# his0si/ConvNet-Quantization

Measured on AMD Instinct MI355X. Metric: images/sec at batch 1024 (3×32×32) int8 static-PTQ, 1/2/4/8 MI355X; top-1 delta, higher is better.
Workload: dtype int8; 1 GPU; full static-PTQ SimpleConvNet, all conv+linear int8 (u8 x s8 -> i32), NHWC, per-tensor weights; global_batch=1024, per_gpu_batch=1024, parallelism=dp1

## Files before the change

### convnet-quantization_amd/csrc/conv3x3.hip

```cpp
#include "common.hpp"
#include "conv_epi.hpp"
#include "conv_launch.hpp"
#include <type_traits>
#include <utility>
#include <algorithm>
#include <cmath>
#include "qconvnet_abi.hpp"

namespace qcn {

constexpr int kPipeD = 2;
constexpr int kSm56D = 4;
constexpr int kProdPrio = 2;

template <int CIN, int COUT, int HW, bool POOL, int WPX, int PSP = 16, int RPAD = 0,
          int SPAD = 0, bool SPLIT = false, int WI_ = 2, int JT_ = 4, int RB_ = 0>
struct ConvCfg {
  static constexpr int kCin = CIN, kCout = COUT;
  static constexpr bool kPool = POOL, kSplit = SPLIT;
  static constexpr int W = HW, H = HW;
  static constexpr int WI = WI_;
  static constexpr int JT = JT_;
  static constexpr int MPS = JT * WI;
  static constexpr int kWpx = WPX;
// ... 1161 lines not shown
      const int PW = C::W / 2, PR = C::R / 2;
      const int q = wp * 32 + (j >> 2) * 16 + p, jq = j & 3;
      return slot(q / (PR * PW), 2 * ((q / PW) % PR) + (jq >> 1), 2 * (q % PW) + (jq & 1));
    }
    const int m = (wp * 8 + j) * 16 + p;
    return slot(m / (C::R * C::W), (m / C::W) % C::R, m % C::W);
  }
  template <class N>
  static constexpr int out_at(int wp, int j, int p) {
    const int m = (wp * 8 + j) * 16 + p;
    return Pix16<N>::slot(m / (C::R * C::W), (m / C::W) % C::R + 1, m % C::W + 1);
  }
  static constexpr int jofs(int j) { return at(0, j, 0) - at(0, 0, 0); }
  template <class N>
  static constexpr int out_jofs(int j) { return out_at<N>(0, j, 0) - out_at<N>(0, 0, 0); }
  static constexpr bool affine() {
    for (int wp = 0; wp < C::kWpx; ++wp)
      for (int j = 0; j < 8; ++j)
        for (int p = 0; p < 16; ++p)
          if (at(wp, j, p) != at(wp, 0, p) + jofs(j)) return false;
    return true;
  }
  template <class N>
  static constexpr bool out_affine() {
    for (int wp = 0; wp < C::kWpx; ++wp)
      for (int j = 0; j < 8; ++j)
        for (int p = 0; p < 16; ++p)
          if (out_at<N>(wp, j, p) != out_at<N>(wp, 0, p) + out_jofs<N>(j)) return false;
    return true;
  }
};

template <class C>
QCN_DEV void pipe_job16(const uint8_t* patch, const int* corr, wt_rsrc_t wr, wt_rsrc_t wrn, int voff, int wc,
                        int lb, int g, v4i (&acc)[4][8], v4i (&ga)[2][4]) {
  constexpr int CBK = C::kCin / 64, S = C::NCH;
  using X = Pix16<C>;
  static_assert(X::affine(), "pixel blocks at constant offsets");
  v4i c0[4];
#pragma unroll
  for (int i = 0; i < 4; ++i) c0[i] = *reinterpret_cast<const v4i*>(corr + wc * 64 + 16 * i + 4 * g);
  auto rd_b = [&](int s, int j) {
    const int tap = s / CBK, cb = s % CBK;
    return *reinterpret_cast<const v4i*>(patch + lb + X::jofs(j) + PatchAddr<C>::delta(tap, j) + cb * 64);
  };
  auto issue = [&](wt_rsrc_t r, int s, int slot) {
#pragma unroll
    for (int i = 0; i < 4; ++i) {
      const auto v = __builtin_amdgcn_raw_buffer_load_b128(r, voff, s * C::WBUF + i * 1024, 0);
      ga[slot][i] = (v4i){(int)v[0], (int)v[1], (int)v[2], (int)v[3]};
    }
  };
  v4i fb[8];
#pragma unroll
  for (int j = 0; j < 8; ++j) fb[j] = rd_b(0, j);
  static_for<S>([&](auto sc) {
    constexpr int s = decltype(sc)::value;
    static_for<32>([&](auto mc) {
      constexpr int m = decltype(mc)::value, j = m >> 2, i = m & 3;
      __builtin_amdgcn_sched_barrier(0);
      acc[i][j] = __builtin_amdgcn_mfma_i32_16x16x64_i8(ga[s & 1][i], fb[j], s == 0 ? c0[i] : acc[i][j], 0, 0, 0);
      __builtin_amdgcn_sched_barrier(0);
      if constexpr (m == 1 && s + 1 < S) {
        issue(wr, s + 1, (s + 1) & 1);
        __builtin_amdgcn_sched_barrier(0);
      }
      if constexpr (i == 3 && s + 1 < S) {
        fb[j] = rd_b(s + 1, j);
        __builtin_amdgcn_sched_barrier(0);
      }
    });
#pragma unroll
    for (int i = 0; i < 4; ++i)
#pragma unroll
      for (int j = 0; j < 8; ++j) asm volatile("" : "+v"(acc[i][j]));
  });
  issue(wrn, 0, 0);
  __builtin_amdgcn_sched_barrier(0);
}

template <class CA, class CB>
struct PairWs16 {
  static_assert(CA::NWAVES == 4 && CB::NWAVES == 4 && CA::WCO == CB::WCO && CA::WI == 2 && CB::WI == 2,
                "four waves of 64-cout x 128-pixel tiles per role");
  static_assert(!CA::kPool && CB::kPool && CA::kCout == CB::kCin, "A feeds B");
  static_assert(CA::PXB == CB::PXB && CA::SEGS == CB::SEGS && CA::R == CA::H && CA::W == CB::W &&
                !CA::kBand && !CB::kBand && !CA::kSplit, "whole images per tile");
  static_assert(Pix16<CA>::affine() && Pix16<CB>::affine() && Pix16<CA>::template out_affine<CB>(),
                "pixel blocks at constant offsets");
  static constexpr int SEGS = CA::SEGS, IMG = CA::IMG;
  static constexpr int IN_BYTES = SEGS * IMG * CA::kCin;
  static_assert(IN_BYTES == 4 * 256 * 16, "four 16-B staging pieces per A-role thread");
  static constexpr int PA = (CA::PATCH + 15) / 16 * 16, PB = (CB::PATCH + 15) / 16 * 16;
  static constexpr int TAB = 16 * (CA::kCout + CB::kCout);
  static constexpr bool DOUBLE_A = 2 * PA + 2 * PB + TAB <= 160 * 1024;
  static constexpr int OFF_PB = 0;
  static constexpr int OFF_PA = 2 * PB;
  static constexpr int OFF_EA = OFF_PA + (DOUBLE_A ? 2 : 1) * PA;
  static constexpr int OFF_EB = OFF_EA + 12 * CA::kCout;
  static constexpr int OFF_CA = OFF_EB + 12 * CB::kCout;
  static constexpr int OFF_CB = OFF_CA + 4 * CA::kCout;
  static constexpr int LDS = OFF_CB + 4 * CB::kCout;
  static_assert(LDS <= 160 * 1024, "LDS budget");
  static constexpr int OPI = CB::OPX / SEGS;
};

template <class CA, class CB, int FA, int FB, bool KMAJOR, bool ILV = false>
QCN_DEV void convpair_ws16_body(int b, int G, const uint8_t* __restrict__ x, int nimg, int x_zp,
                                const int8_t* __restrict__ wa, const ConvEpi& epa, int xb_zp,
                                const int8_t* __restrict__ wb, const ConvEpi& epb, uint8_t* __restrict__ y) {
  using P = PairWs16<CA, CB>;
  using XA = Pix16<CA>;
  using XB = Pix16<CB>;
  constexpr int SEGS = P::SEGS, IMG = CA::IMG, W = CA::W, WCO = CA::WCO;
  constexpr int CH16 = CA::kCin / 16;
  extern __shared__ __attribute__((aligned(16))) uint8_t lds[];
  const int tid = threadIdx.x;
  const int role = __builtin_amdgcn_readfirstlane(tid >> 8);
  const int rt = tid & 255, lane = tid & 63, wave = rt >> 6;
  const int wc = wave % WCO, wp = wave / WCO;
  int T;
  if constexpr (ILV) {
    const int mine = b < nimg ? (nimg - 1 - b) / G + 1 : 0;
    T = (mine + SEGS - 1) / SEGS;
  } else {
    const int ntile = (nimg + SEGS - 1) / SEGS;
    T = b < ntile ? (ntile - 1 - b) / G + 1 : 0;
  }
  auto img_of = [&](int k, int sg) {
    const int n = ILV ? b + (k * SEGS + sg) * G : (b + k * G) * SEGS + sg;
    return n < nimg ? n : (ILV ? b + k * SEGS * G : (b + k * G) * SEGS);
  };
  auto in_src = [&](int k, int q) {
    const int p = rt + 256 * q;
    const int n = img_of(k, p / (IMG * CH16));
    return x + ((long)n * IMG + (p / CH16) % IMG) * CA::kCin + (p % CH16) * 16;
  };
  auto in_dst = [&](int q) {
    const int p = rt + 256 * q;
    const int pix = (p / CH16) % IMG;
    return CA::slot(p / (IMG * CH16), pix / W + 1, pix % W + 1) + (p % CH16) * 16;
  };
  uint4 sv0[4];
  if (role == 0 && T > 0) {
#pragma unroll
    for (int q = 0; q < 4; ++q) sv0[q] = *reinterpret_cast<const uint4*>(in_src(0, q));
  }
  float* eka = reinterpret_cast<float*>(lds + P::OFF_EA);
  float* ekb = reinterpret_cast<float*>(lds + P::OFF_EB);
  int* cra = reinterpret_cast<int*>(lds + P::OFF_CA);
  int* crb = reinterpret_cast<int*>(lds + P::OFF_CB);
  constexpr int NA = 3 * CA::kCout / 4, NB = 3 * CB::kCout / 4;
  constexpr int NCA = CA::kCout / 4, NCB = CB::kCout / 4;
  constexpr int NTAB = NA + NB + NCA + NCB, TPT = (NTAB + 255) / 256;
  float4 tval[TPT];
  auto tab = [&](int e, bool dst) -> float4* {
    if (e < NA) {
      const int a = e / (CA::kCout / 4), o = e % (CA::kCout / 4);
      const float* s = a == 0 ? epa.u : (a == 1 ? epa.v : epa.mult);
      return dst ? reinterpret_cast<float4*>(eka) + e : const_cast<float4*>(reinterpret_cast<const float4*>(s) + o);
    }
    e -= NA;
    if (e < NB) {
      const int a = e / (CB::kCout / 4), o = e % (CB::kCout / 4);
      const float* s = a == 0 ? epb.u : (a == 1 ? epb.v : epb.mult);
      return dst ? reinterpret_cast<float4*>(ekb) + e : const_cast<float4*>(reinterpret_cast<const float4*>(s) + o);
    }
    e -= NB;
    if (e < NCA)
      return dst ? reinterpret_cast<float4*>(cra) + e
                 : const_cast<float4*>(reinterpret_cast<const float4*>(epa.corr) + e);
    e -= NCA;
    return dst ? reinterpret_cast<float4*>(crb) + e
               : const_cast<float4*>(reinterpret_cast<const float4*>(epb.corr) + e);
  };
  {
    const uint32_t pa4 = xor80(splat_u8(x_zp)), pb4 = xor80(splat_u8(xb_zp));
    auto halo = [&](auto cfg, uint8_t* base, int nbuf, int pbytes, uint32_t pad) {
      using C = decltype(cfg);
      constexpr int HS = 2 * C::PCOLS + 2 * (C::PROWS - 2), CH = C::kCin / 16;
      const int total = nbuf * C::SEGS * HS * CH;
      for (int e = tid; e < total; e += 512) {
        const int c = e % CH, hs = (e / CH) % HS, sg = (e / (CH * HS)) % C::SEGS, bf = e / (CH * HS * C::SEGS);
        int pr, pc;
        if (hs < C::PCOLS) { pr = 0; pc = hs; }
        else if (hs < 2 * C::PCOLS) { pr = C::PROWS - 1; pc = hs - C::PCOLS; }
        else { const int r = hs - 2 * C::PCOLS; pr = 1 + (r >> 1); pc = (r & 1) ? C::PCOLS - 1 : 0; }
        *reinterpret_cast<uint4*>(base + bf * pbytes + C::slot(sg, pr, pc) + c * 16) = make_uint4(pad, pad, pad, pad);
      }
    };
    halo(CA{}, lds + P::OFF_PA, P::DOUBLE_A ? 2 : 1, P::PA, pa4);
    halo(CB{}, lds + P::OFF_PB, 2, P::PB, pb4);
  }
  if (role == 1) {
#pragma unroll
    for (int k = 0; k < TPT; ++k)
      if (rt + 256 * k < NTAB) tval[k] = *tab(rt + 256 * k, false);
#pragma unroll
    for (int k = 0; k < TPT; ++k)
      if (rt + 256 * k < NTAB) *tab(rt + 256 * k, true) = tval[k];
  }
  if (T == 0) return;

  const int p16 = lane & 15, g = lane >> 4;
  const wt_rsrc_t wra = wt_rsrc(wa), wrb = wt_rsrc(wb);
  const int voff = (wc * 64 + p16) * 64 + g * 16;
  auto pa_buf = [&](int j) { return lds + P::OFF_PA + (P::DOUBLE_A ? (j & 1) * P::PA : 0); };
  auto pb_buf = [&](int j) { return lds + P::OFF_PB + (j & 1) * P::PB; };
  auto write_in = [&](uint8_t* pa, const uint4 (&sv)[4]) {
#pragma unroll
    for (int q = 0; q < 4; ++q)
      *reinterpret_cast<uint4*>(pa + in_dst(q)) =
          make_uint4(xor80(sv[q].x), xor80(sv[q].y), xor80(sv[q].z), xor80(sv[q].w));
  };
  auto first_chunk = [&](wt_rsrc_t w0, v4i (&ga)[2][4]) {
#pragma unroll
    for (int i = 0; i < 4; ++i) {
      const auto v = __builtin_amdgcn_raw_buffer_load_b128(w0, voff, i * 1024, 0);
      ga[0][i] = (v4i){(int)v[0], (int)v[1], (int)v[2], (int)v[3]};
    }
  };

  v4i acc[4][8];
  if (role == 0) write_in(pa_buf(0), sv0);
  lds_barrier();

  struct Lane {
    int p16, g, ek;
    int la, lb;
    int hb;
    int q;
    const int *ca, *cb;
  };
  auto lanes = [&]() {
    int lz = lane;
    asm volatile("" : "+v"(lz));
    Lane L;
    L.p16 = lz & 15;
    L.g = lz >> 4;
    L.ek = wc * 64 + 4 * L.g;
    L.la = XA::at(wp, 0, L.p16) + 16 * L.g;
    L.lb = XB::at(wp, 0, L.p16) + 16 * L.g;
    L.hb = XA::template out_at<CB>(wp, 0, L.p16) + wc * 64 + 4 * L.g;
    L.q = wp * 32 + L.p16;
    L.ca = cra + (lz >> 6);
    L.cb = crb + (lz >> 6);
    return L;
  };
  auto epi_a = [&](const Lane& L, uint8_t* pb) {
    static_for<4>([&](auto ic) {
      constexpr int i = decltype(ic)::value;
      const EpiG K = load_epig(eka, CA::kCout, L.ek + 16 * i);
      static_for<8>([&](auto jc) {
        constexpr int j = decltype(jc)::value;
        uint32_t wd = 0;
#pragma unroll
        for (int r = 0; r < 4; ++r) wd = rq_elem<FA>(acc[i][j][r], K, r, epa, wd);
        *reinterpret_cast<uint32_t*>(pb + L.hb + XA::template out_jofs<CB>(j) + 16 * i) = xor80(wd);
      });
    });
  };
  auto epi_b = [&](const Lane& L, int k) {
    static_for<2>([&](auto gc) {
      constexpr int gq = decltype(gc)::value;
      uint32_t d[4];
      static_for<4>([&](auto ic) {
        constexpr int i = decltype(ic)::value;
        const EpiG K = load_epig(ekb, CB::kCout, L.ek + 16 * i);
        uint32_t wd = 0;
#pragma unroll
        for (int r = 0; r < 4; ++r) {
          const int a = max(max(acc[i][4 * gq][r], acc[i][4 * gq + 1][r]),
                            max(acc[i][4 * gq + 2][r], acc[i][4 * gq + 3][r]));
          wd = rq_elem<FB>(a, K, r, epb, wd);
        }
        d[i] = wd;
      });
      const auto s02 = __builtin_amdgcn_permlane32_swap(d[0], d[2], false, false);
      const auto s13 = __builtin_amdgcn_permlane32_swap(d[1], d[3], false, false);
      const auto t01 = __builtin_amdgcn_permlane16_swap(s02[0], s13[0], false, false);
      const auto t23 = __builtin_amdgcn_permlane16_swap(s02[1], s13[1], false, false);
      const uint4 v = make_uint4(t01[0], t01[1], t23[0], t23[1]);
      const int q = L.q + 16 * gq;
      const int n = img_of(k, q / P::OPI), pix = q % P::OPI;
      const int co = wc * 64 + 16 * L.g;
      const bool real = ILV ? b + (k * SEGS + q / P::OPI) * G < nimg : (b + k * G) * SEGS + q / P::OPI < nimg;
      if (real) {
        if constexpr (KMAJOR) {
          const int kc = (pix * CB::kCout + co) / 32;
          store_wt16(wt_rsrc(y), (uint32_t)(((long)kc * nimg + n) * 32 + 16 * (L.g & 1)), v);
        } else {
          store_wt16(wt_rsrc(y + (long)n * P::OPI * CB::kCout), (uint32_t)(pix * CB::kCout + co), v);
        }
      }
    });
  };

  if (role == 0) {
    v4i ga[2][4];
    first_chunk(wra, ga);
    uint4 sv[4] = {};
#pragma unroll 1
    for (int p = 0; p <= T; ++p) {
      if constexpr (!P::DOUBLE_A) {
        if (p >= 1 && p < T) write_in(pa_buf(p), sv);
        lds_barrier();
      }
      WS16_STAMP(p, 0);
      if (p < T) {
        const Lane L = lanes();
        pipe_job16<CA>(pa_buf(p), L.ca, wra, wra, voff, wc, L.la, L.g, acc, ga);
        WS16_STAMP(p, 1);
        const int kn = p + 1 < T ? p + 1 : p;
#pragma unroll
        for (int q = 0; q < 4; ++q) sv[q] = *reinterpret_cast<const uint4*>(in_src(kn, q));
        epi_a(L, pb_buf(p));
        if constexpr (P::DOUBLE_A) write_in(pa_buf(p + 1), sv);
        WS16_STAMP(p, 2);
      }
      lds_barrier();
    }
  } else {
    v4i ga[2][4];
    first_chunk(wrb, ga);
#pragma unroll 1
    for (int p = 0; p <= T; ++p) {
      if constexpr (!P::DOUBLE_A) lds_barrier();
      WS16_STAMP(p, 0);
      if (p >= 1) {
        const Lane L = lanes();
        if (p >= 2) epi_b(L, p - 2);
        WS16_STAMP(p, 1);
        pipe_job16<CB>(pb_buf(p - 1), L.cb, wrb, wrb, voff, wc, L.lb, L.g, acc, ga);
        WS16_STAMP(p, 2);
      }
      lds_barrier();
    }
    const Lane L = lanes();
    epi_b(L, T - 1);
#ifdef QCN_CONVNET_STAMP
    if (T + 1 < 8) { WS16_STAMP(T + 1, 0); }
#endif
  }
}

template <class CA, class CB, int FA, int FB, bool KMAJOR>
__global__ __launch_bounds__(512, 1)
void convpair_ws16_kernel(const uint8_t* __restrict__ x, int nimg, int x_zp, const int8_t* __restrict__ wa,
                          ConvEpi epa, int xb_zp, const int8_t* __restrict__ wb, ConvEpi epb,
                          uint8_t* __restrict__ y) {
  convpair_ws16_body<CA, CB, FA, FB, KMAJOR>((int)blockIdx.x, (int)gridDim.x, x, nimg, x_zp, wa, epa, xb_zp,
                                             wb, epb, y);
}

using W16A3 = ConvCfg<64, 128, 16, false, 2, 32, 0, 0, false>;
using W16B4 = ConvCfg<128, 128, 16, true, 2, 32, 64, 0, true>;
using W16A5 = ConvCfg<128, 256, 8, false, 1, 32, 192, 0, false>;
using W16B6 = ConvCfg<256, 256, 8, true, 1, 32, 0, 0, true>;

struct Conv1Cfg {
  static constexpr int H = 32, W = 32, R = 16, COUT = 64, NT = 256;
  static constexpr int PXB = R * W;
  static constexpr int PR = R + 2, PC = W + 2;
  static constexpr int PATCH = 3 * PR * PC;
  static constexpr int PATCH_AL = (PATCH + 15) / 16 * 16;
  static constexpr int KS = 32 + 16;
  static constexpr int LDS = PATCH_AL + PXB * KS;
};

template <int HW>
__global__ __launch_bounds__(256, 3)
void conv1_f32_kernel(const float* __restrict__ x, int nimg, float in_inv, int in_zp,
                      const int8_t* __restrict__ w1, ConvEpi ep, uint8_t* __restrict__ y,
                      uint8_t* __restrict__ qin_out) {
  constexpr int H = HW, W = HW;
// ... 549 lines not shown
                    const int8_t* __restrict__ w1, ConvEpi ep1, int x2_zp,
                    const int8_t* __restrict__ w2, ConvEpi ep2, uint8_t* __restrict__ y) {
  const int T = (int)blockIdx.x < nimg ? 2 * ((nimg - 1 - (int)blockIdx.x) / (int)gridDim.x + 1) : 0;
  conv12p_body((int)blockIdx.x, (int)gridDim.x, T, x, nimg, in_inv, in_zp, w1, ep1, x2_zp, w2, ep2, y);
}
#endif

#define QCN_C16_PARAMS                                                                                   \
  const int8_t* __restrict__ w0, ConvEpi e0, int z0, const int8_t* __restrict__ w1, ConvEpi e1, int z1, \
      const int8_t* __restrict__ w2, ConvEpi e2, int z2, const int8_t* __restrict__ w3, ConvEpi e3,      \
      int z3, const int8_t* __restrict__ w4, ConvEpi e4, int z4, const int8_t* __restrict__ w5,          \
      ConvEpi e5, int z5
#define QCN_C16_ARGS(L)                                                                                  \
  (L).w[0], (L).ep[0], (L).x_zp[0], (L).w[1], (L).ep[1], (L).x_zp[1], (L).w[2], (L).ep[2], (L).x_zp[2],   \
      (L).w[3], (L).ep[3], (L).x_zp[3], (L).w[4], (L).ep[4], (L).x_zp[4], (L).w[5], (L).ep[5], (L).x_zp[5]

struct ConvnetLayers {
  const int8_t* w[6];
  ConvEpi ep[6];
  int x_zp[6];
};

using SmA3 = ConvCfg<64, 128, 16, false, 4, 16, 96, 0, false, 2, 2>;
using SmB4 = ConvCfg<128, 128, 16, true, 2, 16, 32, 0, true, 1, 4>;
using SmA5 = ConvCfg<128, 256, 8, false, 1, 16, 224, 0, false, 1, 2>;
using SmB6 = ConvCfg<256, 256, 8, true, 1, 16, 32, 64, true, 1, 2>;

using WsA3 = ConvCfg<64, 128, 16, false, 2, 16, 96, 0, false>;
using WsB4 = ConvCfg<128, 128, 16, true, 2, 16, 32, 0, true>;
using WsA5 = ConvCfg<128, 256, 8, false, 1, 16, 224, 0, false>;
using WsB6 = ConvCfg<256, 256, 8, true, 1, 16, 32, 64, true>;

constexpr int cmax(int a, int b) { return a > b ? a : b; }
constexpr int kConvnet16Lds = cmax(Conv12P::LDS, cmax(PairWs16<W16A3, W16B4>::LDS, PairWs16<W16A5, W16B6>::LDS));
constexpr int kConvnetSmLds = cmax(Conv12P::LDS, cmax(PairCfg<SmA3, SmB4>::LDS, PairGaCfg<SmA5, SmB6>::LDS));

#ifdef QCN_CONVNET_STAMP
__device__ unsigned long long g_c16_stamp[4096][8];
QCN_DEV void c16_stamp(int i) {
  const unsigned long long t = __builtin_amdgcn_s_memtime();
  const unsigned long long r = __builtin_amdgcn_s_memrealtime();
  const unsigned lane = __builtin_amdgcn_mbcnt_hi(~0u, __builtin_amdgcn_mbcnt_lo(~0u, 0u));
  if ((threadIdx.x >> 6) == 0 && lane == 0 && blockIdx.x < 4096) {
    volatile unsigned long long* d = g_c16_stamp[blockIdx.x];
    d[i] = t + lane;
    d[4 + i] = r + lane;
  }
}
#define C16_STAMP(i) c16_stamp(i)
#else
#define C16_STAMP(i)
#endif

QCN_DEV void phase_boundary() {
  asm volatile("s_waitcnt vmcnt(0) lgkmcnt(0)" ::: "memory");
  __builtin_amdgcn_s_setprio(0);
  __syncthreads();
}

template <int EM, bool KMAJOR>
__global__ __launch_bounds__(512, 1)
void convnet_convs16_kernel(const float* __restrict__ x, int nimg, float in_inv, QCN_C16_PARAMS,
                            uint8_t* __restrict__ a2, uint8_t* __restrict__ a4, uint8_t* __restrict__ a6) {
  static_assert(PairWs16<W16A3, W16B4>::SEGS == 1, "conv3+4 tile k of workgroup b is image b + kG");
  const int b = (int)blockIdx.x, G = (int)gridDim.x;
  const int T = b < nimg ? 2 * ((nimg - 1 - b) / G + 1) : 0;
  C16_STAMP(0);
  conv12p_body(b, G, T, x, nimg, in_inv, z0, w0, e0, z1, w1, e1, a2);
  phase_boundary();
  C16_STAMP(1);
  convpair_ws16_body<W16A3, W16B4, EM, EM, false>(b, G, a2, nimg, z2, w2, e2, z3, w3, e3, a4);
  phase_boundary();
  C16_STAMP(2);
  convpair_ws16_body<W16A5, W16B6, EM, EM, KMAJOR, true>(b, G, a4, nimg, z4, w4, e4, z5, w5, e5, a6);
#ifdef QCN_CONVNET_STAMP
  __syncthreads();
#endif
  C16_STAMP(3);
}

#ifndef QCN_CONV_U8_TU
__global__ __launch_bounds__(512, 1)
void convnet_convs_sm_kernel(const float* __restrict__ x, int nimg, float in_inv, QCN_C16_PARAMS,
                             uint8_t* __restrict__ a2, uint8_t* __restrict__ a4, uint8_t* __restrict__ a6) {
  const int b = (int)blockIdx.x;
  C16_STAMP(0);
  conv12p_body(b, (int)gridDim.x, 2, x, nimg, in_inv, z0, w0, e0, z1, w1, e1, a2);
  phase_boundary();
  C16_STAMP(1);
  convpair_body<SmA3, SmB4>(b, a2, nimg, z2, w2, e2, z3, w3, e3, a4);
  phase_boundary();
  C16_STAMP(2);
  convpair_ga_body<SmA5, SmB6, kSm56D>(b, a4, nimg, z4, w4, e4, z5, w5, e5, a6);
#ifdef QCN_CONVNET_STAMP
  __syncthreads();
#endif
  C16_STAMP(3);
}

struct ConvsF32 {
  static constexpr auto sm = convnet_convs_sm_kernel;
  template <int EM, bool KMAJOR>
  static constexpr auto k16 = convnet_convs16_kernel<EM, KMAJOR>;
  static constexpr int kLdsSm = kConvnetSmLds, kLds16 = kConvnet16Lds;
};
#endif

// ... 494 lines not shown
```

### convnet-quantization_amd/csrc/conv3x3_u8.hip

```cpp
#define QCN_CONV_U8_TU 1
#define QCN_NO_ABI 1
#include "conv3x3.hip"

namespace qcn {

constexpr int kConvnet16LdsU8 = cmax(Conv12P::LDS_U8, kConvnet16Lds);
constexpr int kConvnetSmLdsU8 = cmax(Conv12P::LDS_U8, kConvnetSmLds);

__global__ __launch_bounds__(512, 1)
void conv12p_u8_kernel(const uint8_t* __restrict__ img, int nimg, const uint8_t* __restrict__ qlut,
                       int in_zp, const int8_t* __restrict__ w1, ConvEpi ep1, int x2_zp,
                       const int8_t* __restrict__ w2, ConvEpi ep2, uint8_t* __restrict__ y) {
  const int T = (int)blockIdx.x < nimg ? 2 * ((nimg - 1 - (int)blockIdx.x) / (int)gridDim.x + 1) : 0;
  conv12p_body((int)blockIdx.x, (int)gridDim.x, T, img, nimg, 0.0f, in_zp, w1, ep1, x2_zp, w2, ep2, y,
               qlut);
}

template <int EM, bool KMAJOR>
__global__ __launch_bounds__(512, 1)
void convnet_convs16_u8_kernel(const uint8_t* __restrict__ img, int nimg,
                               const uint8_t* __restrict__ qlut, QCN_C16_PARAMS,
                               uint8_t* __restrict__ a2, uint8_t* __restrict__ a4,
                               uint8_t* __restrict__ a6) {
  static_assert(PairWs16<W16A3, W16B4>::SEGS == 1, "conv3+4 tile k of workgroup b is image b + kG");
  const int b = (int)blockIdx.x, G = (int)gridDim.x;
  const int T = b < nimg ? 2 * ((nimg - 1 - b) / G + 1) : 0;
  conv12p_body(b, G, T, img, nimg, 0.0f, z0, w0, e0, z1, w1, e1, a2, qlut);
  phase_boundary();
  convpair_ws16_body<W16A3, W16B4, EM, EM, false>(b, G, a2, nimg, z2, w2, e2, z3, w3, e3, a4);
  phase_boundary();
  convpair_ws16_body<W16A5, W16B6, EM, EM, KMAJOR, true>(b, G, a4, nimg, z4, w4, e4, z5, w5, e5, a6);
}

__global__ __launch_bounds__(512, 1)
void convnet_convs_sm_u8_kernel(const uint8_t* __restrict__ img, int nimg,
                                const uint8_t* __restrict__ qlut, QCN_C16_PARAMS,
                                uint8_t* __restrict__ a2, uint8_t* __restrict__ a4,
                                uint8_t* __restrict__ a6) {
  const int b = (int)blockIdx.x;
  conv12p_body(b, (int)gridDim.x, 2, img, nimg, 0.0f, z0, w0, e0, z1, w1, e1, a2, qlut);
  phase_boundary();
  convpair_body<SmA3, SmB4>(b, a2, nimg, z2, w2, e2, z3, w3, e3, a4);
  phase_boundary();
  convpair_ga_body<SmA5, SmB6, kSm56D>(b, a4, nimg, z4, w4, e4, z5, w5, e5, a6);
}

struct ConvsU8 {
  static constexpr auto sm = convnet_convs_sm_u8_kernel;
  template <int EM, bool KMAJOR>
  static constexpr auto k16 = convnet_convs16_u8_kernel<EM, KMAJOR>;
  static constexpr int kLdsSm = kConvnetSmLdsU8, kLds16 = kConvnet16LdsU8;
};

}

extern "C" {

int qcn_conv12_fused_u8_nhwc(const uint8_t* img, int nimg, const uint8_t* qlut, int in_zp,
                             const int8_t* w1_packed, const float* u1, const float* v1,
                             const float* mult1, const int32_t* corr1, int z1, int relu1,
                             const qcn_qdq_t* qdq1, int x2_zp, const int8_t* w2_packed,
                             const float* u2, const float* v2, const float* mult2,
                             const int32_t* corr2, int y_zp, int relu2, const qcn_qdq_t* qdq2,
                             uint8_t* y, void* stream) {
// ... 15 lines not shown
```

Measured before the change: 8.473 million images/sec.

## Overlap conv3+4 tail with conv5+6 prologue across the phase seam

```diff
diff --git a/convnet-quantization_amd/csrc/conv3x3.hip b/convnet-quantization_amd/csrc/conv3x3.hip
--- a/convnet-quantization_amd/csrc/conv3x3.hip
+++ b/convnet-quantization_amd/csrc/conv3x3.hip
@@ -1218,7 +1218,7 @@
 
 template <class C>
 QCN_DEV void pipe_job16(const uint8_t* patch, const int* corr, wt_rsrc_t wr, wt_rsrc_t wrn, int voff, int wc,
-                        int lb, int g, v4i (&acc)[4][8], v4i (&ga)[2][4]) {
+                        int lb, int g, v4i (&acc)[4][8], v4i (&ga)[2][4], bool drain = false) {
   constexpr int CBK = C::kCin / 64, S = C::NCH;
   using X = Pix16<C>;
   static_assert(X::affine(), "pixel blocks at constant offsets");
@@ -1260,6 +1260,7 @@
 #pragma unroll
       for (int j = 0; j < 8; ++j) asm volatile("" : "+v"(acc[i][j]));
   });
+  if (drain) asm volatile("s_waitcnt vmcnt(0)" ::: "memory");
   issue(wrn, 0, 0);
   __builtin_amdgcn_sched_barrier(0);
 }
@@ -1290,56 +1291,106 @@
   static constexpr int OPI = CB::OPX / SEGS;
 };
 
-template <class CA, class CB, int FA, int FB, bool KMAJOR, bool ILV = false>
-QCN_DEV void convpair_ws16_body(int b, int G, const uint8_t* __restrict__ x, int nimg, int x_zp,
-                                const int8_t* __restrict__ wa, const ConvEpi& epa, int xb_zp,
-                                const int8_t* __restrict__ wb, const ConvEpi& epb, uint8_t* __restrict__ y) {
+template <class CA, class CB, int FA, int FB, bool KMAJOR, bool ILV = false, int OFF_TAB = PairWs16<CA, CB>::OFF_EA>
+struct Ws16 {
   using P = PairWs16<CA, CB>;
   using XA = Pix16<CA>;
   using XB = Pix16<CB>;
-  constexpr int SEGS = P::SEGS, IMG = CA::IMG, W = CA::W, WCO = CA::WCO;
-  constexpr int CH16 = CA::kCin / 16;
-  extern __shared__ __attribute__((aligned(16))) uint8_t lds[];
-  const int tid = threadIdx.x;
-  const int role = __builtin_amdgcn_readfirstlane(tid >> 8);
-  const int rt = tid & 255, lane = tid & 63, wave = rt >> 6;
-  const int wc = wave % WCO, wp = wave / WCO;
-  int T;
-  if constexpr (ILV) {
-    const int mine = b < nimg ? (nimg - 1 - b) / G + 1 : 0;
-    T = (mine + SEGS - 1) / SEGS;
-  } else {
-    const int ntile = (nimg + SEGS - 1) / SEGS;
-    T = b < ntile ? (ntile - 1 - b) / G + 1 : 0;
-  }
-  auto img_of = [&](int k, int sg) {
+  static constexpr int SEGS = P::SEGS, IMG = CA::IMG, W = CA::W, WCO = CA::WCO;
+  static constexpr int CH16 = CA::kCin / 16;
+  static_assert(OFF_TAB % 16 == 0 && (OFF_TAB == P::OFF_EA || OFF_TAB >= P::LDS) && OFF_TAB + P::TAB <= 160 * 1024,
+                "the tables in their own place or above the phase's patches");
+  static constexpr int OFF_EA = OFF_TAB, OFF_EB = OFF_EA + 12 * CA::kCout, OFF_CA = OFF_EB + 12 * CB::kCout,
+                       OFF_CB = OFF_CA + 4 * CA::kCout;
+  static constexpr int NA = 3 * CA::kCout / 4, NB = 3 * CB::kCout / 4;
+  static constexpr int NCA = CA::kCout / 4, NCB = CB::kCout / 4;
+  static constexpr int NTAB = NA + NB + NCA + NCB, TPT = (NTAB + 255) / 256;
+
+  const int b, G;
+  const uint8_t* const x;
+  const int nimg, x_zp;
+  const ConvEpi& epa;
+  const int xb_zp;
+  const ConvEpi& epb;
+  uint8_t* const y;
+  const wt_rsrc_t wra, wrb;
+  uint8_t* lds;
+  int tid, role, rt, lane, wc, wp, voff, T;
+  float *eka, *ekb;
+  int *cra, *crb;
+
+  QCN_DEV Ws16(int b_, int G_, const uint8_t* x_, int nimg_, int x_zp_, const int8_t* wa, const ConvEpi& epa_,
+               int xb_zp_, const int8_t* wb, const ConvEpi& epb_, uint8_t* y_, bool fresh = false)
+      : b(b_), G(G_), x(x_), nimg(nimg_), x_zp(x_zp_), epa(epa_), xb_zp(xb_zp_), epb(epb_), y(y_),
+        wra(wt_rsrc(wa)), wrb(wt_rsrc(wb)) {
+    extern __shared__ __attribute__((aligned(16))) uint8_t lds_[];
+    lds = lds_;
+    tid = threadIdx.x;
+    if (fresh) asm volatile("" : "+v"(tid));
+    role = __builtin_amdgcn_readfirstlane(tid >> 8);
+    rt = tid & 255, lane = tid & 63;
+    const int wave = rt >> 6;
+    wc = wave % WCO, wp = wave / WCO;
+    voff = (wc * 64 + (lane & 15)) * 64 + (lane >> 4) * 16;
+    if constexpr (ILV) {
+      const int mine = b < nimg ? (nimg - 1 - b) / G + 1 : 0;
+      T = (mine + SEGS - 1) / SEGS;
+    } else {
+      const int ntile = (nimg + SEGS - 1) / SEGS;
+      T = b < ntile ? (ntile - 1 - b) / G + 1 : 0;
+    }
+    eka = reinterpret_cast<float*>(lds + OFF_EA);
+    ekb = reinterpret_cast<float*>(lds + OFF_EB);
+    cra = reinterpret_cast<int*>(lds + OFF_CA);
+    crb = reinterpret_cast<int*>(lds + OFF_CB);
+  }
+
+  QCN_DEV int img_of(int k, int sg) const {
     const int n = ILV ? b + (k * SEGS + sg) * G : (b + k * G) * SEGS + sg;
     return n < nimg ? n : (ILV ? b + k * SEGS * G : (b + k * G) * SEGS);
-  };
-  auto in_src = [&](int k, int q) {
+  }
+  QCN_DEV const uint8_t* in_src(int k, int q) const {
     const int p = rt + 256 * q;
     const int n = img_of(k, p / (IMG * CH16));
     return x + ((long)n * IMG + (p / CH16) % IMG) * CA::kCin + (p % CH16) * 16;
-  };
-  auto in_dst = [&](int q) {
+  }
+  QCN_DEV int in_dst(int q) const {
     const int p = rt + 256 * q;
     const int pix = (p / CH16) % IMG;
     return CA::slot(p / (IMG * CH16), pix / W + 1, pix % W + 1) + (p % CH16) * 16;
-  };
-  uint4 sv0[4];
-  if (role == 0 && T > 0) {
-#pragma unroll
-    for (int q = 0; q < 4; ++q) sv0[q] = *reinterpret_cast<const uint4*>(in_src(0, q));
-  }
-  float* eka = reinterpret_cast<float*>(lds + P::OFF_EA);
-  float* ekb = reinterpret_cast<float*>(lds + P::OFF_EB);
-  int* cra = reinterpret_cast<int*>(lds + P::OFF_CA);
-  int* crb = reinterpret_cast<int*>(lds + P::OFF_CB);
-  constexpr int NA = 3 * CA::kCout / 4, NB = 3 * CB::kCout / 4;
-  constexpr int NCA = CA::kCout / 4, NCB = CB::kCout / 4;
-  constexpr int NTAB = NA + NB + NCA + NCB, TPT = (NTAB + 255) / 256;
-  float4 tval[TPT];
-  auto tab = [&](int e, bool dst) -> float4* {
+  }
+  QCN_DEV void load_in(int k, uint4 (&sv)[4]) const {
+#pragma unroll
+    for (int q = 0; q < 4; ++q) sv[q] = *reinterpret_cast<const uint4*>(in_src(k, q));
+  }
+  QCN_DEV void write_in(uint8_t* pa, const uint4 (&sv)[4]) const {
+#pragma unroll
+    for (int q = 0; q < 4; ++q)
+      *reinterpret_cast<uint4*>(pa + in_dst(q)) =
+          make_uint4(xor80(sv[q].x), xor80(sv[q].y), xor80(sv[q].z), xor80(sv[q].w));
+  }
+  QCN_DEV uint8_t* pa_buf(int j) const { return lds + P::OFF_PA + (P::DOUBLE_A ? (j & 1) * P::PA : 0); }
+  QCN_DEV uint8_t* pb_buf(int j) const { return lds + P::OFF_PB + (j & 1) * P::PB; }
+
+  template <class C>
+  QCN_DEV void halo(uint8_t* base, int nbuf, int pbytes, uint32_t pad, int t, int n) const {
+    constexpr int HS = 2 * C::PCOLS + 2 * (C::PROWS - 2), CH = C::kCin / 16;
+    const int total = nbuf * C::SEGS * HS * CH;
+    for (int e = t; e < total; e += n) {
+      const int c = e % CH, hs = (e / CH) % HS, sg = (e / (CH * HS)) % C::SEGS, bf = e / (CH * HS * C::SEGS);
+      int pr, pc;
+      if (hs < C::PCOLS) { pr = 0; pc = hs; }
+      else if (hs < 2 * C::PCOLS) { pr = C::PROWS - 1; pc = hs - C::PCOLS; }
+      else { const int r = hs - 2 * C::PCOLS; pr = 1 + (r >> 1); pc = (r & 1) ? C::PCOLS - 1 : 0; }
+      *reinterpret_cast<uint4*>(base + bf * pbytes + C::slot(sg, pr, pc) + c * 16) = make_uint4(pad, pad, pad, pad);
+    }
+  }
+  QCN_DEV void halo_a(int t, int n) const {
+    halo<CA>(lds + P::OFF_PA, P::DOUBLE_A ? 2 : 1, P::PA, xor80(splat_u8(x_zp)), t, n);
+  }
+  QCN_DEV void halo_b(int t, int n) const { halo<CB>(lds + P::OFF_PB, 2, P::PB, xor80(splat_u8(xb_zp)), t, n); }
+
+  QCN_DEV float4* tab(int e, bool dst) const {
     if (e < NA) {
       const int a = e / (CA::kCout / 4), o = e % (CA::kCout / 4);
       const float* s = a == 0 ? epa.u : (a == 1 ? epa.v : epa.mult);
@@ -1358,26 +1409,9 @@
     e -= NCA;
     return dst ? reinterpret_cast<float4*>(crb) + e
                : const_cast<float4*>(reinterpret_cast<const float4*>(epb.corr) + e);
-  };
-  {
-    const uint32_t pa4 = xor80(splat_u8(x_zp)), pb4 = xor80(splat_u8(xb_zp));
-    auto halo = [&](auto cfg, uint8_t* base, int nbuf, int pbytes, uint32_t pad) {
-      using C = decltype(cfg);
-      constexpr int HS = 2 * C::PCOLS + 2 * (C::PROWS - 2), CH = C::kCin / 16;
-      const int total = nbuf * C::SEGS * HS * CH;
-      for (int e = tid; e < total; e += 512) {
-        const int c = e % CH, hs = (e / CH) % HS, sg = (e / (CH * HS)) % C::SEGS, bf = e / (CH * HS * C::SEGS);
-        int pr, pc;
-        if (hs < C::PCOLS) { pr = 0; pc = hs; }
-        else if (hs < 2 * C::PCOLS) { pr = C::PROWS - 1; pc = hs - C::PCOLS; }
-        else { const int r = hs - 2 * C::PCOLS; pr = 1 + (r >> 1); pc = (r & 1) ? C::PCOLS - 1 : 0; }
-        *reinterpret_cast<uint4*>(base + bf * pbytes + C::slot(sg, pr, pc) + c * 16) = make_uint4(pad, pad, pad, pad);
-      }
-    };
-    halo(CA{}, lds + P::OFF_PA, P::DOUBLE_A ? 2 : 1, P::PA, pa4);
-    halo(CB{}, lds + P::OFF_PB, 2, P::PB, pb4);
-  }
-  if (role == 1) {
+  }
+  QCN_DEV void tables() const {
+    float4 tval[TPT];
 #pragma unroll
     for (int k = 0; k < TPT; ++k)
       if (rt + 256 * k < NTAB) tval[k] = *tab(rt + 256 * k, false);
@@ -1385,30 +1419,26 @@
     for (int k = 0; k < TPT; ++k)
       if (rt + 256 * k < NTAB) *tab(rt + 256 * k, true) = tval[k];
   }
-  if (T == 0) return;
-
-  const int p16 = lane & 15, g = lane >> 4;
-  const wt_rsrc_t wra = wt_rsrc(wa), wrb = wt_rsrc(wb);
-  const int voff = (wc * 64 + p16) * 64 + g * 16;
-  auto pa_buf = [&](int j) { return lds + P::OFF_PA + (P::DOUBLE_A ? (j & 1) * P::PA : 0); };
-  auto pb_buf = [&](int j) { return lds + P::OFF_PB + (j & 1) * P::PB; };
-  auto write_in = [&](uint8_t* pa, const uint4 (&sv)[4]) {
-#pragma unroll
-    for (int q = 0; q < 4; ++q)
-      *reinterpret_cast<uint4*>(pa + in_dst(q)) =
-          make_uint4(xor80(sv[q].x), xor80(sv[q].y), xor80(sv[q].z), xor80(sv[q].w));
-  };
-  auto first_chunk = [&](wt_rsrc_t w0, v4i (&ga)[2][4]) {
+
+  QCN_DEV bool prologue() const {
+    uint4 sv0[4];
+    if (role == 0 && T > 0) load_in(0, sv0);
+    halo_a(tid, 512);
+    halo_b(tid, 512);
+    if (role == 1) tables();
+    if (T == 0) return false;
+    if (role == 0) write_in(pa_buf(0), sv0);
+    lds_barrier();
+    return true;
+  }
+
+  QCN_DEV void first_chunk(wt_rsrc_t w0, v4i (&ga)[2][4]) const {
 #pragma unroll
     for (int i = 0; i < 4; ++i) {
       const auto v = __builtin_amdgcn_raw_buffer_load_b128(w0, voff, i * 1024, 0);
       ga[0][i] = (v4i){(int)v[0], (int)v[1], (int)v[2], (int)v[3]};
     }
-  };
-
-  v4i acc[4][8];
-  if (role == 0) write_in(pa_buf(0), sv0);
-  lds_barrier();
+  }
 
   struct Lane {
     int p16, g, ek;
@@ -1417,7 +1447,7 @@
     int q;
     const int *ca, *cb;
   };
-  auto lanes = [&]() {
+  QCN_DEV Lane lanes() const {
     int lz = lane;
     asm volatile("" : "+v"(lz));
     Lane L;
@@ -1431,8 +1461,8 @@
     L.ca = cra + (lz >> 6);
     L.cb = crb + (lz >> 6);
     return L;
-  };
-  auto epi_a = [&](const Lane& L, uint8_t* pb) {
+  }
+  QCN_DEV void epi_a(const Lane& L, uint8_t* pb, const v4i (&acc)[4][8]) const {
     static_for<4>([&](auto ic) {
       constexpr int i = decltype(ic)::value;
       const EpiG K = load_epig(eka, CA::kCout, L.ek + 16 * i);
@@ -1444,8 +1474,8 @@
         *reinterpret_cast<uint32_t*>(pb + L.hb + XA::template out_jofs<CB>(j) + 16 * i) = xor80(wd);
       });
     });
-  };
-  auto epi_b = [&](const Lane& L, int k) {
+  }
+  QCN_DEV void epi_b(const Lane& L, int k, const v4i (&acc)[4][8]) const {
     static_for<2>([&](auto gc) {
       constexpr int gq = decltype(gc)::value;
       uint32_t d[4];
@@ -1479,53 +1509,72 @@
         }
       }
     });
-  };
-
-  if (role == 0) {
+  }
+  QCN_DEV void stamp(int p, int k) const { WS16_STAMP(p, k); }
+
+  QCN_DEV void period_a(int p, uint4 (&sv)[4], v4i (&acc)[4][8], v4i (&ga)[2][4], bool seam = false) const {
+    if constexpr (!P::DOUBLE_A) {
+      if (p >= 1 && p < T) write_in(pa_buf(p), sv);
+      lds_barrier();
+    }
+    stamp(p, 0);
+    if (p < T) {
+      const Lane L = lanes();
+      pipe_job16<CA>(pa_buf(p), L.ca, wra, wra, voff, wc, L.la, L.g, acc, ga);
+      stamp(p, 1);
+      load_in(!seam && p + 1 < T ? p + 1 : p, sv);
+      if (seam) lds_barrier();
+      epi_a(L, pb_buf(p), acc);
+      if constexpr (P::DOUBLE_A) write_in(pa_buf(p + 1), sv);
+      stamp(p, 2);
+    }
+    lds_barrier();
+    if (seam) {
+      int k = p + 1 < T ? p + 1 : p;
+      asm volatile("" : "+v"(k));
+      load_in(__builtin_amdgcn_readfirstlane(k), sv);
+    }
+  }
+  QCN_DEV void period_b(int p, v4i (&acc)[4][8], v4i (&ga)[2][4], bool drain = false) const {
+    if constexpr (!P::DOUBLE_A) lds_barrier();
+    stamp(p, 0);
+    if (p >= 1) {
+      const Lane L = lanes();
+      if (p >= 2) epi_b(L, p - 2, acc);
+      stamp(p, 1);
+      pipe_job16<CB>(pb_buf(p - 1), L.cb, wrb, wrb, voff, wc, L.lb, L.g, acc, ga, drain);
+      stamp(p, 2);
+    }
+    lds_barrier();
+  }
+  QCN_DEV void last_epi_b(const v4i (&acc)[4][8]) const {
+    const Lane L = lanes();
+    epi_b(L, T - 1, acc);
+#ifdef QCN_CONVNET_STAMP
+    if (T + 1 < 8) stamp(T + 1, 0);
+#endif
+  }
+};
+
+template <class CA, class CB, int FA, int FB, bool KMAJOR, bool ILV = false>
+QCN_DEV void convpair_ws16_body(int b, int G, const uint8_t* __restrict__ x, int nimg, int x_zp,
+                                const int8_t* __restrict__ wa, const ConvEpi& epa, int xb_zp,
+                                const int8_t* __restrict__ wb, const ConvEpi& epb, uint8_t* __restrict__ y) {
+  const Ws16<CA, CB, FA, FB, KMAJOR, ILV> c(b, G, x, nimg, x_zp, wa, epa, xb_zp, wb, epb, y);
+  if (!c.prologue()) return;
+  v4i acc[4][8];
+  if (c.role == 0) {
     v4i ga[2][4];
-    first_chunk(wra, ga);
+    c.first_chunk(c.wra, ga);
     uint4 sv[4] = {};
 #pragma unroll 1
-    for (int p = 0; p <= T; ++p) {
-      if constexpr (!P::DOUBLE_A) {
-        if (p >= 1 && p < T) write_in(pa_buf(p), sv);
-        lds_barrier();
-      }
-      WS16_STAMP(p, 0);
-      if (p < T) {
-        const Lane L = lanes();
-        pipe_job16<CA>(pa_buf(p), L.ca, wra, wra, voff, wc, L.la, L.g, acc, ga);
-        WS16_STAMP(p, 1);
-        const int kn = p + 1 < T ? p + 1 : p;
-#pragma unroll
-        for (int q = 0; q < 4; ++q) sv[q] = *reinterpret_cast<const uint4*>(in_src(kn, q));
-        epi_a(L, pb_buf(p));
-        if constexpr (P::DOUBLE_A) write_in(pa_buf(p + 1), sv);
-        WS16_STAMP(p, 2);
-      }
-      lds_barrier();
-    }
+    for (int p = 0; p <= c.T; ++p) c.period_a(p, sv, acc, ga);
   } else {
     v4i ga[2][4];
-    first_chunk(wrb, ga);
+    c.first_chunk(c.wrb, ga);
 #pragma unroll 1
-    for (int p = 0; p <= T; ++p) {
-      if constexpr (!P::DOUBLE_A) lds_barrier();
-      WS16_STAMP(p, 0);
-      if (p >= 1) {
-        const Lane L = lanes();
-        if (p >= 2) epi_b(L, p - 2);
-        WS16_STAMP(p, 1);
-        pipe_job16<CB>(pb_buf(p - 1), L.cb, wrb, wrb, voff, wc, L.lb, L.g, acc, ga);
-        WS16_STAMP(p, 2);
-      }
-      lds_barrier();
-    }
-    const Lane L = lanes();
-    epi_b(L, T - 1);
-#ifdef QCN_CONVNET_STAMP
-    if (T + 1 < 8) { WS16_STAMP(T + 1, 0); }
-#endif
+    for (int p = 0; p <= c.T; ++p) c.period_b(p, acc, ga);
+    c.last_epi_b(acc);
   }
 }
 
@@ -2141,7 +2190,28 @@
 using WsB6 = ConvCfg<256, 256, 8, true, 1, 16, 32, 64, true>;
 
 constexpr int cmax(int a, int b) { return a > b ? a : b; }
-constexpr int kConvnet16Lds = cmax(Conv12P::LDS, cmax(PairWs16<W16A3, W16B4>::LDS, PairWs16<W16A5, W16B6>::LDS));
+
+#ifndef QCN_SEAM56
+#define QCN_SEAM56 1
+#endif
+
+struct Seam56 {
+  using P34 = PairWs16<W16A3, W16B4>;
+  using P56 = PairWs16<W16A5, W16B6>;
+  static constexpr int OFF_TAB34 = QCN_SEAM56 ? P56::LDS : P34::OFF_EA;
+  static constexpr int LDS = cmax(P56::LDS, OFF_TAB34 + P34::TAB);
+  static_assert(!P34::DOUBLE_A && !P56::DOUBLE_A, "two barriers per period in both phases");
+  static_assert(P34::SEGS == 1 && P56::SEGS == 2, "conv5+6 tile k is conv3+4 tiles 2 k and 2 k + 1 of the workgroup");
+#if QCN_SEAM56
+  static_assert(P56::OFF_PA >= P34::OFF_PB + 2 * P34::PB, "conv5's patch is above both conv4 buffers");
+  static_assert(P56::OFF_EA == P56::OFF_PA + P56::PA && P56::LDS <= OFF_TAB34,
+                "the conv5+6 patch and tables end below the conv3+4 tables");
+  static_assert(P56::OFF_PB == 0 && 2 * P56::PB <= P56::OFF_PA, "conv6's buffers are below conv5's patch");
+  static_assert(OFF_TAB34 + P34::TAB <= 160 * 1024, "inside the allocation");
+#endif
+};
+
+constexpr int kConvnet16Lds = cmax(Conv12P::LDS, cmax(PairWs16<W16A3, W16B4>::LDS, Seam56::LDS));
 constexpr int kConvnetSmLds = cmax(Conv12P::LDS, cmax(PairCfg<SmA3, SmB4>::LDS, PairGaCfg<SmA5, SmB6>::LDS));
 
 #ifdef QCN_CONVNET_STAMP
@@ -2168,20 +2238,81 @@
 }
 
 template <int EM, bool KMAJOR>
+QCN_DEV void convs36_ws16_body(int b, int G, int nimg, const uint8_t* __restrict__ a2, int z2,
+                               const int8_t* __restrict__ w2, const ConvEpi& e2, int z3,
+                               const int8_t* __restrict__ w3, const ConvEpi& e3, uint8_t* __restrict__ a4, int z4,
+                               const int8_t* __restrict__ w4, const ConvEpi& e4, int z5,
+                               const int8_t* __restrict__ w5, const ConvEpi& e5, uint8_t* __restrict__ a6) {
+#if QCN_SEAM56
+  const Ws16<W16A3, W16B4, EM, EM, false, false, Seam56::OFF_TAB34> c3(b, G, a2, nimg, z2, w2, e2, z3, w3, e3, a4);
+  using C56 = Ws16<W16A5, W16B6, EM, EM, KMAJOR, true>;
+  if (!c3.prologue()) return;
+  const int T3 = c3.T;
+  const bool fused = T3 >= 4;
+  v4i acc[4][8];
+  if (c3.role == 0) {
+    v4i ga[2][4];
+    uint4 sv[4] = {};
+    c3.first_chunk(c3.wra, ga);
+#pragma unroll 1
+    for (int p = 0; p < T3; ++p) c3.period_a(p, sv, acc, ga);
+    const C56 c5(b, G, a4, nimg, z4, w4, e4, z5, w5, e5, a6, true);
+    if (fused) {
+      C16_STAMP(2);
+      c5.load_in(0, sv);
+      c5.halo_a(c5.rt, 256);
+      c5.tables();
+      c5.write_in(c5.pa_buf(0), sv);
+    } else {
+      c3.period_a(T3, sv, acc, ga);
+      phase_boundary();
+      C16_STAMP(2);
+      c5.prologue();
+    }
+    c5.first_chunk(c5.wra, ga);
+#pragma unroll 1
+    for (int p = 0; p <= c5.T; ++p) c5.period_a(p, sv, acc, ga, fused && p == 0);
+  } else {
+    v4i ga[2][4];
+    c3.first_chunk(c3.wrb, ga);
+#pragma unroll 1
+    for (int p = 0; p <= T3; ++p) c3.period_b(p, acc, ga, fused && p == T3 - 1);
+    const C56 c5(b, G, a4, nimg, z4, w4, e4, z5, w5, e5, a6, true);
+    if (fused) c5.first_chunk(c5.wrb, ga);
+    c3.last_epi_b(acc);
+    if (fused) {
+      c5.stamp(0, 0);
+      c5.halo_b(c5.rt, 256);
+      asm volatile("s_waitcnt vmcnt(0)" ::: "memory");
+      lds_barrier();
+    } else {
+      phase_boundary();
+      c5.prologue();
+      c5.first_chunk(c5.wrb, ga);
+    }
+#pragma unroll 1
+    for (int p = fused ? 1 : 0; p <= c5.T; ++p) c5.period_b(p, acc, ga);
+    c5.last_epi_b(acc);
+  }
+#else
+  convpair_ws16_body<W16A3, W16B4, EM, EM, false>(b, G, a2, nimg, z2, w2, e2, z3, w3, e3, a4);
+  phase_boundary();
+  C16_STAMP(2);
+  convpair_ws16_body<W16A5, W16B6, EM, EM, KMAJOR, true>(b, G, a4, nimg, z4, w4, e4, z5, w5, e5, a6);
+#endif
+}
+
+template <int EM, bool KMAJOR>
 __global__ __launch_bounds__(512, 1)
 void convnet_convs16_kernel(const float* __restrict__ x, int nimg, float in_inv, QCN_C16_PARAMS,
                             uint8_t* __restrict__ a2, uint8_t* __restrict__ a4, uint8_t* __restrict__ a6) {
-  static_assert(PairWs16<W16A3, W16B4>::SEGS == 1, "conv3+4 tile k of workgroup b is image b + kG");
   const int b = (int)blockIdx.x, G = (int)gridDim.x;
   const int T = b < nimg ? 2 * ((nimg - 1 - b) / G + 1) : 0;
   C16_STAMP(0);
   conv12p_body(b, G, T, x, nimg, in_inv, z0, w0, e0, z1, w1, e1, a2);
   phase_boundary();
   C16_STAMP(1);
-  convpair_ws16_body<W16A3, W16B4, EM, EM, false>(b, G, a2, nimg, z2, w2, e2, z3, w3, e3, a4);
-  phase_boundary();
-  C16_STAMP(2);
-  convpair_ws16_body<W16A5, W16B6, EM, EM, KMAJOR, true>(b, G, a4, nimg, z4, w4, e4, z5, w5, e5, a6);
+  convs36_ws16_body<EM, KMAJOR>(b, G, nimg, a2, z2, w2, e2, z3, w3, e3, a4, z4, w4, e4, z5, w5, e5, a6);
 #ifdef QCN_CONVNET_STAMP
   __syncthreads();
 #endif
diff --git a/convnet-quantization_amd/csrc/conv3x3_u8.hip b/convnet-quantization_amd/csrc/conv3x3_u8.hip
--- a/convnet-quantization_amd/csrc/conv3x3_u8.hip
+++ b/convnet-quantization_amd/csrc/conv3x3_u8.hip
@@ -22,14 +22,11 @@
                                const uint8_t* __restrict__ qlut, QCN_C16_PARAMS,
                                uint8_t* __restrict__ a2, uint8_t* __restrict__ a4,
                                uint8_t* __restrict__ a6) {
-  static_assert(PairWs16<W16A3, W16B4>::SEGS == 1, "conv3+4 tile k of workgroup b is image b + kG");
   const int b = (int)blockIdx.x, G = (int)gridDim.x;
   const int T = b < nimg ? 2 * ((nimg - 1 - b) / G + 1) : 0;
   conv12p_body(b, G, T, img, nimg, 0.0f, z0, w0, e0, z1, w1, e1, a2, qlut);
   phase_boundary();
-  convpair_ws16_body<W16A3, W16B4, EM, EM, false>(b, G, a2, nimg, z2, w2, e2, z3, w3, e3, a4);
-  phase_boundary();
-  convpair_ws16_body<W16A5, W16B6, EM, EM, KMAJOR, true>(b, G, a4, nimg, z4, w4, e4, z5, w5, e5, a6);
+  convs36_ws16_body<EM, KMAJOR>(b, G, nimg, a2, z2, w2, e2, z3, w3, e3, a4, z4, w4, e4, z5, w5, e5, a6);
 }
 
 __global__ __launch_bounds__(512, 1)
```

New measurement: 8.443 million images/sec. Within noise of the previous version (-0.4%).

## Deepen weight prefetch to two steps and defer next-tile input loads

Applied to the files above, without the earlier changes.

```diff
diff --git a/convnet-quantization_amd/csrc/conv3x3.hip b/convnet-quantization_amd/csrc/conv3x3.hip
--- a/convnet-quantization_amd/csrc/conv3x3.hip
+++ b/convnet-quantization_amd/csrc/conv3x3.hip
@@ -1217,11 +1217,18 @@
 };
 
 template <class C>
+QCN_DEV void ga_issue16(v4i (&ga)[2][4], wt_rsrc_t r, int voff, int s, int slot, int i) {
+  const auto v = __builtin_amdgcn_raw_buffer_load_b128(r, voff, s * C::WBUF + i * 1024, 0);
+  ga[slot][i] = (v4i){(int)v[0], (int)v[1], (int)v[2], (int)v[3]};
+}
+
+template <class C>
 QCN_DEV void pipe_job16(const uint8_t* patch, const int* corr, wt_rsrc_t wr, wt_rsrc_t wrn, int voff, int wc,
                         int lb, int g, v4i (&acc)[4][8], v4i (&ga)[2][4]) {
   constexpr int CBK = C::kCin / 64, S = C::NCH;
   using X = Pix16<C>;
   static_assert(X::affine(), "pixel blocks at constant offsets");
+  static_assert(S >= 3, "steps s and s + 1 in flight while s + 2 is requested");
   v4i c0[4];
 #pragma unroll
   for (int i = 0; i < 4; ++i) c0[i] = *reinterpret_cast<const v4i*>(corr + wc * 64 + 16 * i + 4 * g);
@@ -1229,25 +1236,20 @@
     const int tap = s / CBK, cb = s % CBK;
     return *reinterpret_cast<const v4i*>(patch + lb + X::jofs(j) + PatchAddr<C>::delta(tap, j) + cb * 64);
   };
-  auto issue = [&](wt_rsrc_t r, int s, int slot) {
-#pragma unroll
-    for (int i = 0; i < 4; ++i) {
-      const auto v = __builtin_amdgcn_raw_buffer_load_b128(r, voff, s * C::WBUF + i * 1024, 0);
-      ga[slot][i] = (v4i){(int)v[0], (int)v[1], (int)v[2], (int)v[3]};
-    }
-  };
+#pragma unroll
+  for (int i = 0; i < 4; ++i) ga_issue16<C>(ga, wr, voff, 1, 1, i);
   v4i fb[8];
 #pragma unroll
   for (int j = 0; j < 8; ++j) fb[j] = rd_b(0, j);
   static_for<S>([&](auto sc) {
     constexpr int s = decltype(sc)::value;
     static_for<32>([&](auto mc) {
-      constexpr int m = decltype(mc)::value, j = m >> 2, i = m & 3;
+      constexpr int m = decltype(mc)::value, i = m >> 3, j = m & 7;
       __builtin_amdgcn_sched_barrier(0);
       acc[i][j] = __builtin_amdgcn_mfma_i32_16x16x64_i8(ga[s & 1][i], fb[j], s == 0 ? c0[i] : acc[i][j], 0, 0, 0);
       __builtin_amdgcn_sched_barrier(0);
-      if constexpr (m == 1 && s + 1 < S) {
-        issue(wr, s + 1, (s + 1) & 1);
+      if constexpr (j == 7) {
+        if constexpr (s + 2 < S) ga_issue16<C>(ga, wr, voff, s + 2, s & 1, i);
         __builtin_amdgcn_sched_barrier(0);
       }
       if constexpr (i == 3 && s + 1 < S) {
@@ -1260,7 +1262,8 @@
 #pragma unroll
       for (int j = 0; j < 8; ++j) asm volatile("" : "+v"(acc[i][j]));
   });
-  issue(wrn, 0, 0);
+#pragma unroll
+  for (int i = 0; i < 4; ++i) ga_issue16<C>(ga, wrn, voff, 0, 0, i);
   __builtin_amdgcn_sched_barrier(0);
 }
 
@@ -1302,7 +1305,8 @@
   extern __shared__ __attribute__((aligned(16))) uint8_t lds[];
   const int tid = threadIdx.x;
   const int role = __builtin_amdgcn_readfirstlane(tid >> 8);
-  const int rt = tid & 255, lane = tid & 63, wave = rt >> 6;
+  const int rt = tid & 255, lane = tid & 63;
+  const int wave = __builtin_amdgcn_readfirstlane(rt >> 6);
   const int wc = wave % WCO, wp = wave / WCO;
   int T;
   if constexpr (ILV) {
@@ -1316,12 +1320,12 @@
     const int n = ILV ? b + (k * SEGS + sg) * G : (b + k * G) * SEGS + sg;
     return n < nimg ? n : (ILV ? b + k * SEGS * G : (b + k * G) * SEGS);
   };
-  auto in_src = [&](int k, int q) {
+  auto in_src = [&](int k, int q, int rt) {
     const int p = rt + 256 * q;
     const int n = img_of(k, p / (IMG * CH16));
     return x + ((long)n * IMG + (p / CH16) % IMG) * CA::kCin + (p % CH16) * 16;
   };
-  auto in_dst = [&](int q) {
+  auto in_dst = [&](int q, int rt) {
     const int p = rt + 256 * q;
     const int pix = (p / CH16) % IMG;
     return CA::slot(p / (IMG * CH16), pix / W + 1, pix % W + 1) + (p % CH16) * 16;
@@ -1329,7 +1333,7 @@
   uint4 sv0[4];
   if (role == 0 && T > 0) {
 #pragma unroll
-    for (int q = 0; q < 4; ++q) sv0[q] = *reinterpret_cast<const uint4*>(in_src(0, q));
+    for (int q = 0; q < 4; ++q) sv0[q] = *reinterpret_cast<const uint4*>(in_src(0, q, rt));
   }
   float* eka = reinterpret_cast<float*>(lds + P::OFF_EA);
   float* ekb = reinterpret_cast<float*>(lds + P::OFF_EB);
@@ -1390,20 +1394,23 @@
   const int p16 = lane & 15, g = lane >> 4;
   const wt_rsrc_t wra = wt_rsrc(wa), wrb = wt_rsrc(wb);
   const int voff = (wc * 64 + p16) * 64 + g * 16;
+  auto fresh_rt = [&]() {
+    int t = tid;
+    asm volatile("" : "+v"(t));
+    return t & 255;
+  };
   auto pa_buf = [&](int j) { return lds + P::OFF_PA + (P::DOUBLE_A ? (j & 1) * P::PA : 0); };
   auto pb_buf = [&](int j) { return lds + P::OFF_PB + (j & 1) * P::PB; };
   auto write_in = [&](uint8_t* pa, const uint4 (&sv)[4]) {
+    const int rz = fresh_rt();
 #pragma unroll
     for (int q = 0; q < 4; ++q)
-      *reinterpret_cast<uint4*>(pa + in_dst(q)) =
+      *reinterpret_cast<uint4*>(pa + in_dst(q, rz)) =
           make_uint4(xor80(sv[q].x), xor80(sv[q].y), xor80(sv[q].z), xor80(sv[q].w));
   };
-  auto first_chunk = [&](wt_rsrc_t w0, v4i (&ga)[2][4]) {
-#pragma unroll
-    for (int i = 0; i < 4; ++i) {
-      const auto v = __builtin_amdgcn_raw_buffer_load_b128(w0, voff, i * 1024, 0);
-      ga[0][i] = (v4i){(int)v[0], (int)v[1], (int)v[2], (int)v[3]};
-    }
+  auto first_chunk = [&](auto cfg, wt_rsrc_t w0, v4i (&ga)[2][4]) {
+#pragma unroll
+    for (int i = 0; i < 4; ++i) ga_issue16<decltype(cfg)>(ga, w0, voff, 0, 0, i);
   };
 
   v4i acc[4][8];
@@ -1432,7 +1439,7 @@
     L.cb = crb + (lz >> 6);
     return L;
   };
-  auto epi_a = [&](const Lane& L, uint8_t* pb) {
+  auto epi_a = [&](const Lane& L, uint8_t* pb, auto&& after_first) {
     static_for<4>([&](auto ic) {
       constexpr int i = decltype(ic)::value;
       const EpiG K = load_epig(eka, CA::kCout, L.ek + 16 * i);
@@ -1443,6 +1450,11 @@
         for (int r = 0; r < 4; ++r) wd = rq_elem<FA>(acc[i][j][r], K, r, epa, wd);
         *reinterpret_cast<uint32_t*>(pb + L.hb + XA::template out_jofs<CB>(j) + 16 * i) = xor80(wd);
       });
+      if constexpr (i == 0) {
+        __builtin_amdgcn_sched_barrier(0);
+        after_first();
+        __builtin_amdgcn_sched_barrier(0);
+      }
     });
   };
   auto epi_b = [&](const Lane& L, int k) {
@@ -1483,7 +1495,7 @@
 
   if (role == 0) {
     v4i ga[2][4];
-    first_chunk(wra, ga);
+    first_chunk(CA{}, wra, ga);
     uint4 sv[4] = {};
 #pragma unroll 1
     for (int p = 0; p <= T; ++p) {
@@ -1496,10 +1508,11 @@
         const Lane L = lanes();
         pipe_job16<CA>(pa_buf(p), L.ca, wra, wra, voff, wc, L.la, L.g, acc, ga);
         WS16_STAMP(p, 1);
-        const int kn = p + 1 < T ? p + 1 : p;
-#pragma unroll
-        for (int q = 0; q < 4; ++q) sv[q] = *reinterpret_cast<const uint4*>(in_src(kn, q));
-        epi_a(L, pb_buf(p));
+        epi_a(L, pb_buf(p), [&]() {
+          const int kn = p + 1 < T ? p + 1 : p, rz = fresh_rt();
+#pragma unroll
+          for (int q = 0; q < 4; ++q) sv[q] = *reinterpret_cast<const uint4*>(in_src(kn, q, rz));
+        });
         if constexpr (P::DOUBLE_A) write_in(pa_buf(p + 1), sv);
         WS16_STAMP(p, 2);
       }
@@ -1507,7 +1520,7 @@
     }
   } else {
     v4i ga[2][4];
-    first_chunk(wrb, ga);
+    first_chunk(CB{}, wrb, ga);
 #pragma unroll 1
     for (int p = 0; p <= T; ++p) {
       if constexpr (!P::DOUBLE_A) lds_barrier();
```

Measured after the change: 8.365 million images/sec before, 8.487 million images/sec after, median of 6. 1.01x the previous value.
